# alexkeroro86/SampleNeRFRO

Hardware: AMD Instinct MI355X
Metric: rays/sec (train step) (higher is better)
Workload: dtype f16x3/fp32-acc

## Files before the change

samplenerfro_amd/csrc/mlp.hip:

```cpp
#include "common.h"
#include "nerfmlp_layout.h"
#include "mfma_ops.h"
#include "bkgd_layout.h"
#include "so3_layout.h"

#include <stdlib.h>
#include <type_traits>
#include <vector>
#include <stdio.h>

namespace rnerf {


#define GLOBAL_AS __attribute__((address_space(1)))
#define LDS_AS __attribute__((address_space(3)))

struct MfmaLayer { int dense, ks, nt, kind; };
__host__ __device__ constexpr MfmaLayer mfma_layer(int l) {
  constexpr MfmaLayer t[10] = {{0, 4, 8, 0},  {1, 16, 8, 1}, {2, 16, 8, 1}, {3, 16, 8, 1}, {4, 16, 8, 1},
                               {5, 20, 8, 2}, {6, 16, 8, 1}, {7, 16, 8, 1}, {9, 16, 8, 1}, {10, 18, 4, 3}};
  return t[l];
}
__host__ __device__ constexpr int layer_blocks_before(int l) {
  int o = 0;
// ... 374 lines not shown
template <int PREC, bool MASK, bool ONE = false>
struct SeamWork {
  f32x16 (&acc0)[8];
  f32x16 (&acc1)[8];
  f32x16 (&prev0)[8];
  float4* st1;
  PrevConv<PREC, 0, MASK, true, ONE> cv;
  __device__ __forceinline__ SeamWork(f32x16 (&a0)[8], f32x16 (&a1)[8], f32x16 (&p0)[8], float4* s1) : acc0(a0), acc1(a1), prev0(p0), st1(s1), cv(a0[0]) {}
  template <int C, int T>
  __device__ __forceinline__ void move() {
    if constexpr (C == 0) prev0[T] = acc0[T];
    else if constexpr (!ONE) st1[(T * 4 + C - 1) * 64] = make_float4(acc1[T][4 * (C - 1)], acc1[T][4 * (C - 1) + 1], acc1[T][4 * (C - 1) + 2], acc1[T][4 * (C - 1) + 3]);
  }
  template <int C, int Q>
  __device__ __forceinline__ void conv() {
    if constexpr (ONE && Q >= 4) return;
    if constexpr (C == 0 && Q >= 4) { cv.v1[2 * (Q & 3)] = acc1[0][2 * (Q & 3)]; cv.v1[2 * (Q & 3) + 1] = acc1[0][2 * (Q & 3) + 1]; }
    cv.template chunk<C, Q>();
  }
  template <int C, int PI>
  __device__ __forceinline__ void chunk() {
    if constexpr (PI >= 1) {
      move<C, PI - 1>();
      conv<C, PI - 1>();
      if constexpr (PI == 7 && C == 4) { conv<0, 7>(); conv<1, 7>(); conv<2, 7>(); conv<3, 7>(); conv<4, 7>(); }
    }
  }
  __device__ __forceinline__ void finish() {
    move<0, 7>(); move<1, 7>(); move<2, 7>(); move<3, 7>(); move<4, 7>();
  }
};


template <int PREC, bool FIRST, int PI, typename W, int PASSES = Prec<PREC>::PASSES, typename BOPS = KOps>
__device__ __forceinline__ void tile_mfma(f32x16& a0, f32x16& a1, const uint4 ah, const uint4 al, const BOPS& b, W& work) {
  using PP = Prec<PREC>;
  constexpr bool TWO = !BOPS::ONE;
  const f32x16 zero = {0, 0, 0, 0, 0, 0, 0, 0, 0, 0, 0, 0, 0, 0, 0, 0};
  a0 = mfma16<PP::F16>(ah, b.h0, FIRST ? zero : a0);
  work.template chunk<0, PI>();
  RNERF_PIN();
  if constexpr (TWO) a1 = mfma16<PP::F16>(ah, b.h1, FIRST ? zero : a1);
  work.template chunk<1, PI>();
  RNERF_PIN();
  if constexpr (PP::NP == 2 && PASSES == 3) {
    a0 = mfma16<PP::F16>(ah, b.l0, a0);
    work.template chunk<2, PI>();
    RNERF_PIN();
    if constexpr (TWO) a1 = mfma16<PP::F16>(ah, b.l1, a1);
    work.template chunk<3, PI>();
    RNERF_PIN();
    a0 = mfma16<PP::F16>(al, b.h0, a0);
    work.template chunk<4, PI>();
    RNERF_PIN();
    if constexpr (TWO) a1 = mfma16<PP::F16>(al, b.h1, a1);
  } else if constexpr (PP::NP == 2 && PASSES == 38) {
    a0 = mfma_f8(al.x, al.y, b.l0.x, b.l0.y, a0);
    work.template chunk<2, PI>();
    RNERF_PIN();
    if constexpr (TWO) a1 = mfma_f8(al.x, al.y, b.l1.x, b.l1.y, a1);
    work.template chunk<3, PI>();
    RNERF_PIN();
    a0 = mfma_f8(al.z, al.w, b.l0.z, b.l0.w, a0);
    work.template chunk<4, PI>();
    RNERF_PIN();
    if constexpr (TWO) a1 = mfma_f8(al.z, al.w, b.l1.z, b.l1.w, a1);
  } else if constexpr (PP::NP == 2 && PASSES == 2) {
    a0 = mfma16<PP::F16>(ah, b.l0, a0);
    work.template chunk<2, PI>();
    work.template chunk<3, PI>();
    RNERF_PIN();
    if constexpr (TWO) a1 = mfma16<PP::F16>(ah, b.l1, a1);
    work.template chunk<4, PI>();
  } else if constexpr (PP::NP == 2 && PASSES == 22) {
    a0 = mfma16<PP::F16>(al, b.h0, a0);
    work.template chunk<2, PI>();
    work.template chunk<3, PI>();
    RNERF_PIN();
    if constexpr (TWO) a1 = mfma16<PP::F16>(al, b.h1, a1);
    work.template chunk<4, PI>();
  } else {
    work.template chunk<2, PI>();
    work.template chunk<3, PI>();
    work.template chunk<4, PI>();
  }
  RNERF_PIN();
}

struct NoDma { __device__ __forceinline__ void operator()() const {} };

constexpr int FRAG_DEPTH = 4;

template <int PREC, int NT, int KOFF, bool FIRST, typename W, typename D = NoDma, int PASSES = Prec<PREC>::PASSES, typename BOPS = KOps>
__device__ __forceinline__ void kstep_mfma(f32x16 (&acc0)[8], f32x16 (&acc1)[8], const BOPS& b, const char* slab, int lane, W& work, D dma = D()) {
  using PP = Prec<PREC>;
  const uint4* a = (const uint4*)slab + lane + (size_t)KOFF * NT * PP::NP * 64;
  uint4 fh[FRAG_DEPTH], fl[FRAG_DEPTH];
  auto load_lo = [&](int tile) -> uint4 {
    if constexpr (PP::F8X) {
      const uint2* a2 = (const uint2*)((const uint4*)slab + ((size_t)KOFF * NT + tile) * PP::NP * 64 + 64) + lane;
      const uint2 u = a2[0], v = a2[64];
      return make_uint4(u.x, u.y, v.x, v.y);
    } else return a[(tile * PP::NP + PP::NP - 1) * 64];
  };
#pragma unroll
  for (int t = 0; t < FRAG_DEPTH; ++t) {
    const int tt = t < NT ? t : NT - 1;
    fh[t] = a[(tt * PP::NP) * 64];
    fl[t] = load_lo(tt);
  }
#define RNERF_TILE(T)                                                                                     \
  if constexpr (T < NT) {                                                                                 \
    const uint4 ah = fh[T % FRAG_DEPTH], al = fl[T % FRAG_DEPTH];                                         \
    tile_mfma<PREC, FIRST, (T & 7), W, PASSES, BOPS>(acc0[T], acc1[T], ah, al, b, work);                  \
    if constexpr (T + FRAG_DEPTH < NT) {                                                                  \
      fh[T % FRAG_DEPTH] = a[((T + FRAG_DEPTH) * PP::NP) * 64];                                           \
      fl[T % FRAG_DEPTH] = load_lo(T + FRAG_DEPTH);                                                       \
    }                                                                                                     \
  }
  RNERF_TILE(0) RNERF_TILE(1)
  dma();
  RNERF_TILE(2)
  if constexpr (NT == 8) RNERF_PIN();
  RNERF_TILE(3)
  if constexpr (NT == 8) RNERF_PIN();
  RNERF_TILE(4)
  if constexpr (NT == 8) RNERF_PIN();
  RNERF_TILE(5)
  if constexpr (NT == 8) RNERF_PIN();
  RNERF_TILE(6) RNERF_TILE(7)
#undef RNERF_TILE
}

constexpr int SAVE_PE = 0, SAVE_L1 = 4, SAVE_VIEW = 148, SAVE_RGBIN = 150, SAVE_SLOTS = 158, SAVE_MASK = 158, SAVE_TOTAL = 167;
__host__ __device__ constexpr size_t sv_mask0(long long R) { return (size_t)(R / 32) * SAVE_SLOTS * 64; }
__host__ __device__ constexpr size_t sv_lo0(long long R) { return sv_mask0(R) + (size_t)(R / 32) * 576; }
__host__ __device__ constexpr size_t sv_addr(int q, long long t32, int m, int h) { return (((size_t)t32 * SAVE_SLOTS + q) * 32 + m) * 2 + h; }
__host__ __device__ constexpr size_t sv_mask_addr(int sw, long long t32, int m, int h) { return (((size_t)t32 * 36 + sw) * 32 + m) * 2 + h; }

__device__ __forceinline__ uint32_t nz_nibbles(const uint4& o) {
  return pk_min1(o.x) | (pk_min1(o.y) << 1) | (pk_min1(o.z) << 2) | (pk_min1(o.w) << 3);
}
__device__ __forceinline__ uint32_t nz_byte(uint32_t nib) { return (nib & 0xFu) | (nib >> 12); }

template <int PREC, int MODE, int TRAIN, bool ONE = false>
__global__ void __launch_bounds__(256, 1)
nerfmlp_fwd_kernel(const char* __restrict__ packed, const float4* __restrict__ rows_pd, const float4* __restrict__ rows_dr,
// ... 44 lines not shown
      return n_tiles;
    } else {
      return t;
    }
  };
  const int first_tile = find_next((int)blockIdx.x);
  if (first_tile < n_tiles) { issue_slab<SLAB>(packed, 0u, wave, lane); off = SLAB; }
  slab_wait_dma();
  __syncthreads();

  for (int tile = first_tile; tile < n_tiles;) {
    if (tileq != nullptr && tid == 0)
      __hip_atomic_store(tileq + 1 + blockIdx.x, (int)gridDim.x + atomicAdd(tileq, 1), __ATOMIC_RELAXED, __HIP_MEMORY_SCOPE_AGENT);
    const float* __restrict__ auxt = aux;
    asm volatile("" : "+s"(auxt));
    int next_tile = n_tiles;
    long long row[2]; bool row_ok[2];
    float4 pd[2], dr[2];
#pragma unroll
    for (int mt = 0; mt < 2; ++mt) {
      if (ONE && mt == 1) { row[1] = row[0]; row_ok[1] = false; pd[1] = pd[0]; dr[1] = dr[0]; continue; }
      row[mt] = (long long)tile * TROWS + wave * WROWS + mt * 32 + m;
      row_ok[mt] = row[mt] < total_rows;
      if (!row_ok[mt]) row[mt] = total_rows - 1;
      size_t rec = (size_t)row[mt];
      if (node_of_sample) { const long long sidx = row[mt] / B; rec = (size_t)node_of_sample[sidx] * B + (size_t)(row[mt] - sidx * B); }
      pd[mt] = rows_pd[rec];
      dr[mt] = rows_dr[rec];
    }

    f32x16 acc0[8], acc1[8], prev0[8];

    const long long t32_0 = (long long)tile * (TROWS / 32) + wave * (WROWS / 32);
    auto save_ops = [&](int q, const KOps& o) {
      if constexpr (TRAIN != 0) {
        uint4* dst = save + sv_addr(q, t32_0, m, h);
        stream_store(dst, o.h0);
        if constexpr (!ONE) stream_store(dst + (size_t)SAVE_SLOTS * 64, o.h1);
        if constexpr (TRAIN == 2) {
          uint4* dl = dst + sv_lo0(save_rows);
          stream_store(dl, o.l0);
          if constexpr (!ONE) stream_store(dl + (size_t)SAVE_SLOTS * 64, o.l1);
        }
        if constexpr (TRAIN == 3) {
          uint2* dl = (uint2*)(save + sv_lo0(save_rows)) + sv_addr(q, t32_0, m, h);
          stream_store8(dl, lo8_pack<false>(o.l0, LO8_SCALE_X));
          if constexpr (!ONE) stream_store8(dl + (size_t)SAVE_SLOTS * 64, lo8_pack<false>(o.l1, LO8_SCALE_X));
        }
      }
    };

    uint32_t ovf0 = 0, ovf1 = 0;
    auto watch = [&](const KOps& o, bool is_signed) {
      const uint32_t am = is_signed ? 0x7FFF7FFFu : 0xFFFFFFFFu;
      ovf0 = pk_maxu(pk_maxu(ovf0, o.h0.x & am), pk_maxu(pk_maxu(o.h0.y & am, o.h0.z & am), o.h0.w & am));
      if constexpr (!ONE) ovf1 = pk_maxu(pk_maxu(ovf1, o.h1.x & am), pk_maxu(pk_maxu(o.h1.y & am, o.h1.z & am), o.h1.w & am));
    };

    uint32_t mw0 = 0, mw1 = 0;
    auto save_mask = [&](int set, int s, uint32_t nib0, uint32_t nib1) {
      if constexpr (TRAIN != 0) {
        if ((s & 3) == 0) { mw0 = nz_byte(nib0); mw1 = nz_byte(nib1); }
        else { mw0 |= nz_byte(nib0) << (8 * (s & 3)); mw1 |= nz_byte(nib1) << (8 * (s & 3)); }
        if ((s & 3) == 3) {
          uint32_t* dst = (uint32_t*)(save + sv_mask0(save_rows)) + sv_mask_addr(set * 4 + (s >> 2), t32_0, m, h);
          __builtin_nontemporal_store(mw0, dst);
          if constexpr (!ONE) __builtin_nontemporal_store(mw1, dst + 36 * 64);
        }
      }
    };

    auto enc_ops = [&](const float4 (&v)[2], int s, int nsin) -> KOps {
      const float phase = h ? 1.5707963705062866f : 0.0f;
      float f[2][8];
#pragma unroll
      for (int mt = 0; mt < (ONE ? 1 : 2); ++mt)
#pragma unroll
        for (int j = 0; j < 8; ++j) {
          const int q = 8 * s + j;
          if (q < nsin) {
            const int d = q / 3, c = q % 3;
            const float x = c == 0 ? v[mt].x : (c == 1 ? v[mt].y : v[mt].z);
            f[mt][j] = pe_sin(fadd(fmul(x, (float)(1 << d)), phase));
// ... 23 lines not shown
      }
      KOps o;
      split8<PREC>(x0, o.h0, o.l0);
      if constexpr (ONE) { o.h1 = o.h0; o.l1 = o.l0; } else split8<PREC>(x1, o.h1, o.l1);
      return o;
    };

    auto load_bias8 = [&](int s, const float* __restrict__ bias, float (&b)[8]) {
      const float4 b0 = *(const float4*)(bias + 16 * s + 4 * h), b1 = *(const float4*)(bias + 16 * s + 8 + 4 * h);
      b[0] = b0.x; b[1] = b0.y; b[2] = b0.z; b[3] = b0.w; b[4] = b1.x; b[5] = b1.y; b[6] = b1.z; b[7] = b1.w;
    };
    auto load_state8 = [&](int s, float (&v)[8]) {
      if constexpr (ONE) return;
      const float4 u0 = st1[((s >> 1) * 4 + 2 * (s & 1)) * 64], u1 = st1[((s >> 1) * 4 + 2 * (s & 1) + 1) * 64];
      v[0] = u0.x; v[1] = u0.y; v[2] = u0.z; v[3] = u0.w; v[4] = u1.x; v[5] = u1.y; v[6] = u1.z; v[7] = u1.w;
    };
    NoWork nowork;

#define SLAB_PREFETCH(DO_NEXT)                                                                                       \
  do { if (DO_NEXT) { issue_slab<SLAB>(packed + off, (unsigned)((buf ^ 1) * SLAB), wave, lane); off += SLAB; } } while (0)
#define SLAB_DONE() do { slab_wait_dma(); __syncthreads(); buf ^= 1; } while (0)

    float sig0 = 0.f, sig1 = 0.f;

    KOps cur;
    {
      cur = enc_ops(pd, 0, 30);
      SeamWork<PREC, TRAIN != 0, ONE> seam(acc0, acc1, prev0, st1);
      seam.cv.floor_v = RELU_FLOOR;
      load_bias8(0, auxt + AUX_BIAS, seam.cv.b);
      load_bias8(0, auxt + AUX_ZERO, seam.cv.ws);
#define RNERF_PE_KSTEP(S, FIRST_, SAVE_)                                                                             \
      {                                                                                                              \
        if (SAVE_) save_ops(SAVE_PE + S, cur);                                                                       \
        watch(cur, true);          \
        SLAB_PREFETCH(true);    \
        if constexpr (S < 3) {                                                                                       \
          EncWork<PREC, S + 1, 30, ONE> ew(pd, h);                                                                        \
          kstep_mfma<PREC, 8, 0, FIRST_>(acc0, acc1, cur, smem + buf * SLAB, lane, ew);                              \
          cur = ew.result();                                                                                         \
        } else {                                                                                                     \
          kstep_mfma<PREC, 8, 0, false>(acc0, acc1, cur, smem + buf * SLAB, lane, seam);                             \
        }                                                                                                            \
        SLAB_DONE();                                                                                                 \
      }
      RNERF_PE_KSTEP(0, true, true) RNERF_PE_KSTEP(1, false, true) RNERF_PE_KSTEP(2, false, true) RNERF_PE_KSTEP(3, false, true)
      seam.finish();
      cur = seam.cv.result();
    }

    float bnext[8], wnext[8];
    load_bias8(1, auxt + AUX_BIAS, bnext);
    load_bias8(1, auxt + AUX_ZERO, wnext);

#pragma unroll 1
    for (int l = 1; l <= 8; ++l) {
      const float* __restrict__ bias = auxt + AUX_BIAS + 256 * (l - 1);
      SeamWork<PREC, TRAIN != 0, ONE> seam(acc0, acc1, prev0, st1);
      seam.cv.floor_v = l == 8 ? NO_FLOOR : RELU_FLOOR;
      const float* __restrict__ wseam = auxt + (l == 7 ? AUX_WSIG : AUX_ZERO);
      const float* __restrict__ wsel = auxt + (l == 8 ? AUX_WSIG : AUX_ZERO);
#define RNERF_KSTEP(S)                                                                                              \
      {                                                                                                              \
        save_ops(SAVE_L1 + 16 * (l - 1) + S, cur);                                                                   \
        watch(cur, false);                                                                                           \
        if constexpr (TRAIN != 0 && S == 0) save_mask(l - 1, 0, nz_nibbles(cur.h0), nz_nibbles(cur.h1));                  \
        if constexpr (S == 13) { load_bias8(0, bias + 256, seam.cv.b); load_bias8(0, wseam, seam.cv.ws); }           \
        float bnn[8], wnn[8];                                                                                        \
        if constexpr (S + 2 < 16) { load_bias8(S + 2, bias, bnn); load_bias8(S + 2, wsel, wnn); }    \
        else if constexpr (S == 14) { load_bias8(1, bias + 256, bnn); load_bias8(1, wseam, wnn); }    \
        auto dma = [&]() { SLAB_PREFETCH(true); };                                                                   \
        if constexpr (S + 1 < 16) {                                                                                  \
          PrevConv<PREC, S + 1, TRAIN != 0, true, ONE> cv(prev0[(S + 1) >> 1]);                                           \
          cv.floor_v = RELU_FLOOR;                                                                                        \
          _Pragma("unroll") for (int j = 0; j < 8; ++j) { cv.b[j] = bnext[j]; cv.ws[j] = wnext[j]; }                 \
          load_state8(S + 1, cv.v1);                                                                                 \
          kstep_mfma<PREC, 8, 0, S == 0, PrevConv<PREC, S + 1, TRAIN != 0, true, ONE>, decltype(dma)>(acc0, acc1, cur, smem + buf * SLAB, lane, cv, dma); \
          cur = cv.result();                                                                                         \
          sig0 += cv.sg0; sig1 += cv.sg1;                                                                            \
          save_mask(l - 1, S + 1, cv.nz[0], cv.nz[1]);                                                               \
        } else {                                                                                                     \
           \
           \
          kstep_mfma<PREC, 8, 0, false, SeamWork<PREC, TRAIN != 0, ONE>, decltype(dma)>(acc0, acc1, cur, smem + buf * SLAB, lane, seam, dma); \
        }                                                                                                            \
        if constexpr (S + 2 <= 16) { _Pragma("unroll") for (int j = 0; j < 8; ++j) { bnext[j] = bnn[j]; wnext[j] = wnn[j]; } } \
        SLAB_DONE();                                                                                                 \
      }
      RNERF_KSTEP(0) RNERF_KSTEP(1) RNERF_KSTEP(2) RNERF_KSTEP(3) RNERF_KSTEP(4) RNERF_KSTEP(5) RNERF_KSTEP(6) RNERF_KSTEP(7)
      RNERF_KSTEP(8) RNERF_KSTEP(9) RNERF_KSTEP(10) RNERF_KSTEP(11) RNERF_KSTEP(12) RNERF_KSTEP(13) RNERF_KSTEP(14) RNERF_KSTEP(15)
#undef RNERF_KSTEP
      if (l == 5) {
        asm volatile("" : "+v"(pd[0].x), "+v"(pd[0].y), "+v"(pd[0].z), "+v"(pd[1].x), "+v"(pd[1].y), "+v"(pd[1].z));
        cur = enc_ops(pd, 0, 30);
        RNERF_PE_KSTEP(0, false, false) RNERF_PE_KSTEP(1, false, false) RNERF_PE_KSTEP(2, false, false) RNERF_PE_KSTEP(3, false, false)
      }
      seam.finish();
      cur = seam.cv.result();
      sig0 += seam.cv.sg0; sig1 += seam.cv.sg1;
    }

    {
      const float* __restrict__ bias = auxt + AUX_BIAS + 256 * 8;
      KOps c0 = cur;
      KOps c1 = prev_ops(1, bias, NO_FLOOR);
      float bA[8], bB[8];
      load_bias8(2, bias, bA);
      load_bias8(3, bias, bB);
#define RNERF_VSLAB(SL)                                                                                              \
      {                                                                                                              \
        save_ops(SAVE_L1 + 16 * 8 + 2 * SL, c0);                                                                     \
        save_ops(SAVE_L1 + 16 * 8 + 2 * SL + 1, c1);                                                                 \
        watch(c0, true); watch(c1, true);                                                                            \
        SLAB_PREFETCH(true);                                                                                         \
        if constexpr (SL + 1 < 8) {                                                                                  \
          float bA2[8], bB2[8];                                                                                      \
          if constexpr (SL + 2 < 8) { load_bias8(2 * SL + 4, bias, bA2); load_bias8(2 * SL + 5, bias, bB2); }        \
          PrevConv<PREC, 2 * SL + 2, false, false, ONE> cvA(prev0[SL + 1]);                                                      \
          PrevConv<PREC, 2 * SL + 3, false, false, ONE> cvB(prev0[SL + 1]);                                                      \
          cvA.floor_v = NO_FLOOR; cvB.floor_v = NO_FLOOR;                                                                \
          _Pragma("unroll") for (int j = 0; j < 8; ++j) { cvA.b[j] = bA[j]; cvB.b[j] = bB[j]; }                      \
          load_state8(2 * SL + 2, cvA.v1);                                                                           \
          load_state8(2 * SL + 3, cvB.v1);                                                                           \
          PairOfPairs<decltype(cvA)> wA(cvA);                                                                        \
          PairOfPairs<decltype(cvB)> wB(cvB);                                                                        \
          kstep_mfma<PREC, 4, 0, SL == 0>(acc0, acc1, c0, smem + buf * SLAB, lane, wA);                              \
          kstep_mfma<PREC, 4, 1, false>(acc0, acc1, c1, smem + buf * SLAB, lane, wB);                                \
          c0 = cvA.result(); c1 = cvB.result();                                                                      \
          if constexpr (SL + 2 < 8) { _Pragma("unroll") for (int j = 0; j < 8; ++j) { bA[j] = bA2[j]; bB[j] = bB2[j]; } } \
        } else {                                                                                                     \
          const KOps n0 = enc_ops(dr, 0, 12), n1 = enc_ops(dr, 1, 12);                                               \
          kstep_mfma<PREC, 4, 0, false>(acc0, acc1, c0, smem + buf * SLAB, lane, nowork);                            \
          kstep_mfma<PREC, 4, 1, false>(acc0, acc1, c1, smem + buf * SLAB, lane, nowork);                            \
          c0 = n0; c1 = n1;                                                                                          \
        }                                                                                                            \
        SLAB_DONE();                                                                                                 \
      }
      RNERF_VSLAB(0) RNERF_VSLAB(1) RNERF_VSLAB(2) RNERF_VSLAB(3) RNERF_VSLAB(4) RNERF_VSLAB(5) RNERF_VSLAB(6) RNERF_VSLAB(7)
#undef RNERF_VSLAB
      save_ops(SAVE_VIEW, c0);
      save_ops(SAVE_VIEW + 1, c1);
      watch(c0, true); watch(c1, true);
      next_tile = tileq != nullptr ? __builtin_amdgcn_readfirstlane(__hip_atomic_load(tileq + 1 + blockIdx.x, __ATOMIC_RELAXED, __HIP_MEMORY_SCOPE_AGENT))
                                   : find_next(tile + (int)gridDim.x);
      const bool has_next_tile = next_tile < n_tiles;
      if (has_next_tile) off = 0;
      SLAB_PREFETCH(has_next_tile);
      kstep_mfma<PREC, 4, 0, false>(acc0, acc1, c0, smem + buf * SLAB, lane, nowork);
      kstep_mfma<PREC, 4, 1, false>(acc0, acc1, c1, smem + buf * SLAB, lane, nowork);
      SLAB_DONE();
    }

    {
      const float* __restrict__ hw = auxt + 4 * h;
      auto head_load = [&](int t, float4 (&W)[16]) {
#pragma unroll
        for (int g = 0; g < 4; ++g) {
          const int n = 32 * t + 8 * g;
          W[4 * g] = gload4(hw + AUX_BIAS + 256 * 9 + n);
          W[4 * g + 1] = gload4(hw + AUX_WRGB + n); W[4 * g + 2] = gload4(hw + AUX_WRGB + 128 + n); W[4 * g + 3] = gload4(hw + AUX_WRGB + 256 + n);
        }
      };
      float p0[3] = {0.f, 0.f, 0.f}, p1[3] = {0.f, 0.f, 0.f};
      float4 Wc[16];
      head_load(0, Wc);
#pragma unroll
      for (int t = 0; t < 4; ++t) {
        float4 Wn[16];
        if (t + 1 < 4) head_load(t + 1, Wn);
        RNERF_PIN();
        float rv0[16], rv1[16];
#pragma unroll
        for (int g = 0; g < 4; ++g) {
          const float4 bb = Wc[4 * g], wr = Wc[4 * g + 1], wg = Wc[4 * g + 2], wb = Wc[4 * g + 3];
          const float bv[4] = {bb.x, bb.y, bb.z, bb.w}, wrv[4] = {wr.x, wr.y, wr.z, wr.w}, wgv[4] = {wg.x, wg.y, wg.z, wg.w}, wbv[4] = {wb.x, wb.y, wb.z, wb.w};
#pragma unroll
          for (int i = 0; i < 4; ++i) {
            const float v0 = relu_keep(fmaf(acc0[t][4 * g + i], INV_SCALE, bv[i]), RELU_FLOOR);
            p0[0] = fmaf(v0, wrv[i], p0[0]); p0[1] = fmaf(v0, wgv[i], p0[1]); p0[2] = fmaf(v0, wbv[i], p0[2]);
            rv0[4 * g + i] = v0;
            if constexpr (!ONE) {
              const float v1 = relu_keep(fmaf(acc1[t][4 * g + i], INV_SCALE, bv[i]), RELU_FLOOR);
// ... 174 lines not shown
  int buf = 0;
  size_t off = 0;
  NoWork nowork;

  if ((int)blockIdx.x < n_tiles) { issue_slab<SLAB>(packed_bwd, 0u, wave, lane); off = SLAB; }
  slab_wait_dma();
  __syncthreads();

  float mref = 0.f;
  for (int tile = blockIdx.x; tile < n_tiles; tile += gridDim.x) {
    const bool has_next_tile = tile + (int)gridDim.x < n_tiles;
    const long long srow0 = (long long)tile * TROWS + wave * WROWS + m;
    const long long t32_0 = (long long)tile * (TROWS / 32) + wave * (WROWS / 32);
    float4 g[2];
#pragma unroll
    for (int mt = 0; mt < 2; ++mt) {
      if (ONE && mt == 1) { g[1] = make_float4(0.f, 0.f, 0.f, 0.f); continue; }
      const long long row = srow0 + 32 * mt;
      g[mt] = row < total_rows ? d_raw[row] : make_float4(0.f, 0.f, 0.f, 0.f);
      if constexpr (BW::F16) {
        const float mx = fmaxf(fmaxf(fabsf(g[mt].x), fabsf(g[mt].y)), fmaxf(fabsf(g[mt].z), fabsf(g[mt].w)));
        const uint32_t ex = __builtin_bit_cast(uint32_t, mx) >> 23;
        const bool okx = ex >= 8 && ex <= 250;
        const float m_row = okx ? __builtin_bit_cast(float, (ex - 5) << 23) : 0.0f;
        const float inv = okx ? __builtin_bit_cast(float, (259 - ex) << 23) : 0.0f;
        g[mt].x *= inv; g[mt].y *= inv; g[mt].z *= inv; g[mt].w *= inv;
        float* rs = (float*)(dy + dy_plane_uint4(save_rows, BW::NP));
        if (h == 0) rs[row] = m_row;
        mref = fmaxf(mref, m_row);
      }
    }
    f32x16 acc0[8], acc1[8], prev0[8];

    auto dy_store = [&](int q, const KOps& o) {
      uint4* dst = dy + dy_addr(q, t32_0, m, h);
      stream_store(dst, o.h0);
      if constexpr (!ONE) stream_store(dst + (size_t)DY_SLOTS * 64, o.h1);
      if constexpr (BW::LO8) {
        uint2* dl = (uint2*)(dy + dy_plane_uint4(save_rows, 1)) + dy_addr(q, t32_0, m, h);
        stream_store8(dl, lo8_pack<true>(o.l0, LO8_SCALE_D));
        if constexpr (!ONE) stream_store8(dl + (size_t)DY_SLOTS * 64, lo8_pack<true>(o.l1, LO8_SCALE_D));
      } else if constexpr (BW::NP == 2) {
        uint4* dl = dst + dy_plane_uint4(save_rows, 1);
        stream_store(dl, o.l0);
        if constexpr (!ONE) stream_store(dl + (size_t)DY_SLOTS * 64, o.l1);
      }
    };
    auto mask_at = [&](int set, uint4& a, uint4& b) {
      const uint32_t* src = (const uint32_t*)(saved + sv_mask0(save_rows)) + sv_mask_addr(set * 4, t32_0, m, h);
      constexpr size_t ws = 64, mt1 = 36 * 64;
#define RNERF_NTL(P) __builtin_nontemporal_load(P)
      a = make_uint4(RNERF_NTL(src), RNERF_NTL(src + ws), RNERF_NTL(src + 2 * ws), RNERF_NTL(src + 3 * ws));
      if constexpr (ONE) b = make_uint4(0, 0, 0, 0);
      else b = make_uint4(RNERF_NTL(src + mt1), RNERF_NTL(src + ws + mt1), RNERF_NTL(src + 2 * ws + mt1), RNERF_NTL(src + 3 * ws + mt1));
#undef RNERF_NTL
    };
    auto grad_ops = [&](int s, bool use_mask, const uint4 mk0, const uint4 mk1, const float* __restrict__ wadd) -> KOps {
      float r1[8] = {0.f, 0.f, 0.f, 0.f, 0.f, 0.f, 0.f, 0.f};
      if constexpr (!ONE) {
        const float4 u0 = st1[((s >> 1) * 4 + 2 * (s & 1)) * 64], u1 = st1[((s >> 1) * 4 + 2 * (s & 1) + 1) * 64];
        r1[0] = u0.x; r1[1] = u0.y; r1[2] = u0.z; r1[3] = u0.w; r1[4] = u1.x; r1[5] = u1.y; r1[6] = u1.z; r1[7] = u1.w;
      }
      const uint32_t w0 = (s >> 2) == 0 ? mk0.x : ((s >> 2) == 1 ? mk0.y : ((s >> 2) == 2 ? mk0.z : mk0.w));
      const uint32_t w1 = (s >> 2) == 0 ? mk1.x : ((s >> 2) == 1 ? mk1.y : ((s >> 2) == 2 ? mk1.z : mk1.w));
      float x0[8], x1[8];
#pragma unroll
      for (int j = 0; j < 8; ++j) {
        float a = prev0[s >> 1][8 * (s & 1) + j] * INV_SCALE, b = r1[j] * INV_SCALE;
        if (wadd) { const float w = wadd[16 * s + 8 * (j >> 2) + 4 * h + (j & 3)]; a = fmaf(g[0].w, w, a); b = fmaf(g[1].w, w, b); }
        if (use_mask) {
          const uint32_t bit = 1u << (8 * (s & 3) + (j >> 1) + 4 * (j & 1));
          a = (w0 & bit) ? a : 0.f;
          b = (w1 & bit) ? b : 0.f;
        }
        x0[j] = a; x1[j] = b;
      }
      KOps o;
      if constexpr (ONE) { split8<PREC>(x0, o.h0, o.l0); if constexpr (!(NEED_LO || BW::NP == 2)) o.l0 = make_uint4(0, 0, 0, 0); o.h1 = o.h0; o.l1 = o.l0; }
      else if constexpr (NEED_LO || BW::NP == 2) { split8<PREC>(x0, o.h0, o.l0); split8<PREC>(x1, o.h1, o.l1); }
// ... 19 lines not shown
  do { if (DO_NEXT) { issue_slab<SLAB>(packed_bwd + off, (unsigned)((buf ^ 1) * SLAB), wave, lane); off += SLAB; } } while (0)
#define SLAB_DONE() do { slab_wait_dma(); __syncthreads(); buf ^= 1; } while (0)

    {
      KOps o;
      float hz0[8] = {0, 0, 0, 0, 0, 0, 0, 0}, hz1[8] = {0, 0, 0, 0, 0, 0, 0, 0};
      if (h == 0) { hz0[0] = g[0].w; hz0[1] = g[0].x; hz0[2] = g[0].y; hz0[3] = g[0].z; hz1[0] = g[1].w; hz1[1] = g[1].x; hz1[2] = g[1].y; hz1[3] = g[1].z; }
      split8<PREC>(hz0, o.h0, o.l0);
      if constexpr (ONE) { o.h1 = o.h0; o.l1 = o.l0; } else split8<PREC>(hz1, o.h1, o.l1);
      dy_store(DY_HEADS, o);
#pragma unroll
      for (int t = 0; t < 8; ++t)
#pragma unroll
        for (int r = 0; r < 16; ++r) {
          float a = 0.f, b = 0.f;
          if (t < 4) {
            const int n = 32 * t + (r & 3) + 8 * (r >> 2) + 4 * h;
            const float wr = fwd_aux[AUX_WRGB + n], wg = fwd_aux[AUX_WRGB + 128 + n], wb = fwd_aux[AUX_WRGB + 256 + n];
            a = (g[0].x * wr + g[0].y * wg + g[0].z * wb) * PP::WSCALE;
            b = (g[1].x * wr + g[1].y * wg + g[1].z * wb) * PP::WSCALE;
          }
          acc0[t][r] = a;
          if constexpr (!ONE) acc1[t][r] = b;
        }
      layer_end();
    }

    {
      uint4 ma, mb;
      mask_at(8, ma, mb);
      KOps cur = grad_ops(0, true, ma, mb, nullptr);
#define RNERF_DG_KSTEP(S, NSTEPS, SLOT0, PREFETCH_STMT)                                                                       \
      {                                                                                                                         \
        dy_store((SLOT0) + S, cur);                                                                                             \
        auto dma = [&]() { PREFETCH_STMT; };    \
        if constexpr (S + 1 < NSTEPS) {                                                                                         \
          GradConv<PREC, S + 1, NEED_LO, ONE> cv(prev0[(S + 1) >> 1]);                                                                   \
          if constexpr (!ONE) {                                                                                                 \
            const float4 u0 = st1[(((S + 1) >> 1) * 4 + 2 * ((S + 1) & 1)) * 64], u1 = st1[(((S + 1) >> 1) * 4 + 2 * ((S + 1) & 1) + 1) * 64]; \
            cv.v1[0] = u0.x; cv.v1[1] = u0.y; cv.v1[2] = u0.z; cv.v1[3] = u0.w; cv.v1[4] = u1.x; cv.v1[5] = u1.y; cv.v1[6] = u1.z; cv.v1[7] = u1.w; \
          }                                                                                                                     \
          if (wadd) {            \
            const float4 wa = *(const float4*)(wadd + 16 * (S + 1) + 4 * h), wb = *(const float4*)(wadd + 16 * (S + 1) + 8 + 4 * h); \
            const float wv[8] = {wa.x, wa.y, wa.z, wa.w, wb.x, wb.y, wb.z, wb.w};                                               \
            _Pragma("unroll") for (int j = 0; j < 8; ++j) { cv.t0[j] = g[0].w * wv[j]; cv.t1[j] = g[1].w * wv[j]; }             \
          } else {                                                                                                              \
            _Pragma("unroll") for (int j = 0; j < 8; ++j) { cv.t0[j] = 0.f; cv.t1[j] = 0.f; }                                   \
          }                                                                                                                     \
          cv.w0 = ((S + 1) >> 2) == 0 ? ma.x : (((S + 1) >> 2) == 1 ? ma.y : (((S + 1) >> 2) == 2 ? ma.z : ma.w));             \
          cv.w1 = ((S + 1) >> 2) == 0 ? mb.x : (((S + 1) >> 2) == 1 ? mb.y : (((S + 1) >> 2) == 2 ? mb.z : mb.w));             \
          kstep_mfma<PREC, 8, 0, S == 0, GradConv<PREC, S + 1, NEED_LO, ONE>, decltype(dma), DGP>(acc0, acc1, cur, smem + buf * SLAB, lane, cv, dma); \
          cur = cv.result();                                                                                                    \
        } else {                                                                                                                \
          kstep_mfma<PREC, 8, 0, false, NoWork, decltype(dma), DGP>(acc0, acc1, cur, smem + buf * SLAB, lane, nowork, dma);         \
        }                                                                                                                       \
        SLAB_DONE();                                                                                                            \
      }
      {
        const float* __restrict__ wadd = nullptr;
        RNERF_DG_KSTEP(0, 8, DY_L9, SLAB_PREFETCH(true)) RNERF_DG_KSTEP(1, 8, DY_L9, SLAB_PREFETCH(true))
        RNERF_DG_KSTEP(2, 8, DY_L9, SLAB_PREFETCH(true)) RNERF_DG_KSTEP(3, 8, DY_L9, SLAB_PREFETCH(true))
        RNERF_DG_KSTEP(4, 8, DY_L9, SLAB_PREFETCH(true)) RNERF_DG_KSTEP(5, 8, DY_L9, SLAB_PREFETCH(true))
        RNERF_DG_KSTEP(6, 8, DY_L9, SLAB_PREFETCH(true)) RNERF_DG_KSTEP(7, 8, DY_L9, SLAB_PREFETCH(true))
      }
      layer_end();
    }

    uint4 nma = make_uint4(0, 0, 0, 0), nmb = nma;
#pragma unroll 1
    for (int l = 8; l >= 1; --l) {
      const bool use_mask = l != 8;
      const float* __restrict__ wadd = (l == 7) ? fwd_aux + AUX_WSIG : nullptr;
      uint4 ma = nma, mb = nmb;
      if (!use_mask) { ma = make_uint4(~0u, ~0u, ~0u, ~0u); mb = ma; }
      mask_at(l - 1, nma, nmb);
      KOps cur = grad_ops(0, true, ma, mb, wadd);
      const int slot0 = 16 * l;
#define RNERF_DG_PF(S) do { if ((S) == 15 && l == 1) { if (has_next_tile) off = 0; SLAB_PREFETCH(has_next_tile); } else SLAB_PREFETCH(true); } while (0)
      RNERF_DG_KSTEP(0, 16, slot0, RNERF_DG_PF(0)) RNERF_DG_KSTEP(1, 16, slot0, RNERF_DG_PF(1)) RNERF_DG_KSTEP(2, 16, slot0, RNERF_DG_PF(2))
      RNERF_DG_KSTEP(3, 16, slot0, RNERF_DG_PF(3)) RNERF_DG_KSTEP(4, 16, slot0, RNERF_DG_PF(4)) RNERF_DG_KSTEP(5, 16, slot0, RNERF_DG_PF(5))
      RNERF_DG_KSTEP(6, 16, slot0, RNERF_DG_PF(6)) RNERF_DG_KSTEP(7, 16, slot0, RNERF_DG_PF(7)) RNERF_DG_KSTEP(8, 16, slot0, RNERF_DG_PF(8))
      RNERF_DG_KSTEP(9, 16, slot0, RNERF_DG_PF(9)) RNERF_DG_KSTEP(10, 16, slot0, RNERF_DG_PF(10)) RNERF_DG_KSTEP(11, 16, slot0, RNERF_DG_PF(11))
      RNERF_DG_KSTEP(12, 16, slot0, RNERF_DG_PF(12)) RNERF_DG_KSTEP(13, 16, slot0, RNERF_DG_PF(13)) RNERF_DG_KSTEP(14, 16, slot0, RNERF_DG_PF(14))
      RNERF_DG_KSTEP(15, 16, slot0, RNERF_DG_PF(15))
#undef RNERF_DG_PF
      layer_end();
    }
// ... 1913 lines not shown
```

Baseline: 673,900.

## Stagger activation save stores across MFMA slots, one wave per slot

Instead of issuing all operand/gradient save stores for a k-step as a burst before the MFMA sequence, the stores are split into parts and scheduled at distinct MFMA positions inside the k-step. Each part is issued by only one wave, chosen by MFMA position, so the waves take turns rather than all storing at the same time. A static check keeps a store from sharing a slot with the weight DMA. The aim is to spread global write traffic across the matrix pipeline and reduce store-queue stalls. The cost is more template machinery and a different per-lane address computation, and correctness depends on every store part landing at some slot.

Result: slower. 643,100 (-4.6%).

```diff
diff --git a/samplenerfro_amd/csrc/mlp.hip b/samplenerfro_amd/csrc/mlp.hip
--- a/samplenerfro_amd/csrc/mlp.hip
+++ b/samplenerfro_amd/csrc/mlp.hip
@@ -430,52 +430,87 @@
 };
 
 
-template <int PREC, bool FIRST, int PI, typename W, int PASSES = Prec<PREC>::PASSES, typename BOPS = KOps>
-__device__ __forceinline__ void tile_mfma(f32x16& a0, f32x16& a1, const uint4 ah, const uint4 al, const BOPS& b, W& work) {
+struct NoSave {
+  template <int POS, int M> static constexpr bool stores_at() { return false; }
+  template <int POS, int M> __device__ __forceinline__ void at() const {}
+};
+template <int J> struct StorePart { static constexpr int value = J; };
+template <int NS, typename F>
+struct StaggeredSave {
+  const int wave;
+  const F store;
+  __device__ __forceinline__ StaggeredSave(int wave_, const F& store_) : wave(wave_), store(store_) {}
+  template <int POS, int M> static constexpr bool stores_at() { return POS % (M / NS / 4) == 0 && (POS % (M / NS)) / (M / NS / 4) < 4; }
+  template <int POS, int M> __device__ __forceinline__ void at() const {
+    static_assert(M % NS == 0 && M / NS >= 4, "fewer than four MFMAs per store");
+    if constexpr (stores_at<POS, M>()) {
+      if (wave == (POS % (M / NS)) / (M / NS / 4)) store(StorePart<POS / (M / NS)>());
+    }
+  }
+};
+template <int NS, typename F>
+__device__ __forceinline__ StaggeredSave<NS, F> staggered_save(int wave, const F& store) { return StaggeredSave<NS, F>(wave, store); }
+
+template <int PREC, int PASSES, bool ONE>
+constexpr int tile_mfmas() {
+  constexpr int per = Prec<PREC>::NP != 2 ? 1 : ((PASSES == 3 || PASSES == 38) ? 3 : ((PASSES == 2 || PASSES == 22) ? 2 : 1));
+  return per * (ONE ? 1 : 2);
+}
+
+template <int PREC, bool FIRST, int PI, typename W, int PASSES = Prec<PREC>::PASSES, typename BOPS = KOps, typename SV = NoSave, int T = 0, int NT = 8>
+__device__ __forceinline__ void tile_mfma(f32x16& a0, f32x16& a1, const uint4 ah, const uint4 al, const BOPS& b, W& work, const SV& sv = SV()) {
   using PP = Prec<PREC>;
   constexpr bool TWO = !BOPS::ONE;
+  constexpr int MPT = tile_mfmas<PREC, PASSES, BOPS::ONE>(), M = NT * MPT, P0 = T * MPT, ST = TWO ? 2 : 1;
   const f32x16 zero = {0, 0, 0, 0, 0, 0, 0, 0, 0, 0, 0, 0, 0, 0, 0, 0};
   a0 = mfma16<PP::F16>(ah, b.h0, FIRST ? zero : a0);
+  sv.template at<P0, M>();
   work.template chunk<0, PI>();
   RNERF_PIN();
-  if constexpr (TWO) a1 = mfma16<PP::F16>(ah, b.h1, FIRST ? zero : a1);
+  if constexpr (TWO) { a1 = mfma16<PP::F16>(ah, b.h1, FIRST ? zero : a1); sv.template at<P0 + 1, M>(); }
   work.template chunk<1, PI>();
   RNERF_PIN();
   if constexpr (PP::NP == 2 && PASSES == 3) {
     a0 = mfma16<PP::F16>(ah, b.l0, a0);
+    sv.template at<P0 + ST, M>();
     work.template chunk<2, PI>();
     RNERF_PIN();
-    if constexpr (TWO) a1 = mfma16<PP::F16>(ah, b.l1, a1);
+    if constexpr (TWO) { a1 = mfma16<PP::F16>(ah, b.l1, a1); sv.template at<P0 + 3, M>(); }
     work.template chunk<3, PI>();
     RNERF_PIN();
     a0 = mfma16<PP::F16>(al, b.h0, a0);
+    sv.template at<P0 + 2 * ST, M>();
     work.template chunk<4, PI>();
     RNERF_PIN();
-    if constexpr (TWO) a1 = mfma16<PP::F16>(al, b.h1, a1);
+    if constexpr (TWO) { a1 = mfma16<PP::F16>(al, b.h1, a1); sv.template at<P0 + 5, M>(); }
   } else if constexpr (PP::NP == 2 && PASSES == 38) {
     a0 = mfma_f8(al.x, al.y, b.l0.x, b.l0.y, a0);
+    sv.template at<P0 + ST, M>();
     work.template chunk<2, PI>();
     RNERF_PIN();
-    if constexpr (TWO) a1 = mfma_f8(al.x, al.y, b.l1.x, b.l1.y, a1);
+    if constexpr (TWO) { a1 = mfma_f8(al.x, al.y, b.l1.x, b.l1.y, a1); sv.template at<P0 + 3, M>(); }
     work.template chunk<3, PI>();
     RNERF_PIN();
     a0 = mfma_f8(al.z, al.w, b.l0.z, b.l0.w, a0);
+    sv.template at<P0 + 2 * ST, M>();
     work.template chunk<4, PI>();
     RNERF_PIN();
-    if constexpr (TWO) a1 = mfma_f8(al.z, al.w, b.l1.z, b.l1.w, a1);
+    if constexpr (TWO) { a1 = mfma_f8(al.z, al.w, b.l1.z, b.l1.w, a1); sv.template at<P0 + 5, M>(); }
   } else if constexpr (PP::NP == 2 && PASSES == 2) {
     a0 = mfma16<PP::F16>(ah, b.l0, a0);
+    sv.template at<P0 + ST, M>();
     work.template chunk<2, PI>();
     work.template chunk<3, PI>();
     RNERF_PIN();
-    if constexpr (TWO) a1 = mfma16<PP::F16>(ah, b.l1, a1);
+    if constexpr (TWO) { a1 = mfma16<PP::F16>(ah, b.l1, a1); sv.template at<P0 + 3, M>(); }
     work.template chunk<4, PI>();
   } else if constexpr (PP::NP == 2 && PASSES == 22) {
     a0 = mfma16<PP::F16>(al, b.h0, a0);
+    sv.template at<P0 + ST, M>();
     work.template chunk<2, PI>();
     work.template chunk<3, PI>();
     RNERF_PIN();
-    if constexpr (TWO) a1 = mfma16<PP::F16>(al, b.h1, a1);
+    if constexpr (TWO) { a1 = mfma16<PP::F16>(al, b.h1, a1); sv.template at<P0 + 3, M>(); }
     work.template chunk<4, PI>();
   } else {
     work.template chunk<2, PI>();
@@ -486,12 +521,13 @@
 }
 
 struct NoDma { __device__ __forceinline__ void operator()() const {} };
-
 constexpr int FRAG_DEPTH = 4;
 
-template <int PREC, int NT, int KOFF, bool FIRST, typename W, typename D = NoDma, int PASSES = Prec<PREC>::PASSES, typename BOPS = KOps>
-__device__ __forceinline__ void kstep_mfma(f32x16 (&acc0)[8], f32x16 (&acc1)[8], const BOPS& b, const char* slab, int lane, W& work, D dma = D()) {
+template <int PREC, int NT, int KOFF, bool FIRST, typename W, typename D = NoDma, int PASSES = Prec<PREC>::PASSES, typename BOPS = KOps, typename SV = NoSave>
+__device__ __forceinline__ void kstep_mfma(f32x16 (&acc0)[8], f32x16 (&acc1)[8], const BOPS& b, const char* slab, int lane, W& work, D dma = D(), const SV& sv = SV()) {
   using PP = Prec<PREC>;
+  static_assert(std::is_same<D, NoDma>::value || !SV::template stores_at<2 * tile_mfmas<PREC, PASSES, BOPS::ONE>() - 1, NT * tile_mfmas<PREC, PASSES, BOPS::ONE>()>(),
+                "an operand save shares its place with the weight DMA");
   const uint4* a = (const uint4*)slab + lane + (size_t)KOFF * NT * PP::NP * 64;
   uint4 fh[FRAG_DEPTH], fl[FRAG_DEPTH];
   auto load_lo = [&](int tile) -> uint4 {
@@ -510,7 +546,7 @@
 #define RNERF_TILE(T)                                                                                     \
   if constexpr (T < NT) {                                                                                 \
     const uint4 ah = fh[T % FRAG_DEPTH], al = fl[T % FRAG_DEPTH];                                         \
-    tile_mfma<PREC, FIRST, (T & 7), W, PASSES, BOPS>(acc0[T], acc1[T], ah, al, b, work);                  \
+    tile_mfma<PREC, FIRST, (T & 7), W, PASSES, BOPS, SV, T, NT>(acc0[T], acc1[T], ah, al, b, work, sv);   \
     if constexpr (T + FRAG_DEPTH < NT) {                                                                  \
       fh[T % FRAG_DEPTH] = a[((T + FRAG_DEPTH) * PP::NP) * 64];                                           \
       fl[T % FRAG_DEPTH] = load_lo(T + FRAG_DEPTH);                                                       \
@@ -621,23 +657,25 @@
     f32x16 acc0[8], acc1[8], prev0[8];
 
     const long long t32_0 = (long long)tile * (TROWS / 32) + wave * (WROWS / 32);
+    const unsigned lane16_ = (unsigned)(m * 2 + h) * 16u;
+    constexpr int SAVE_MT = ONE ? 1 : 2, SAVE_NS = SAVE_MT * (TRAIN >= 2 ? 2 : 1);
+    auto save_part = [&](int q, const KOps& o, auto J) {
+      constexpr int plane = decltype(J)::value / SAVE_MT, mt = decltype(J)::value % SAVE_MT;
+      if constexpr (TRAIN != 0) {
+        const size_t blk = sv_addr(q, t32_0 + mt, 0, 0);
+        unsigned lane16 = lane16_;
+        asm volatile("" : "+v"(lane16));
+        if constexpr (plane == 0) stream_store((uint4*)((char*)(save + blk) + lane16), mt ? o.h1 : o.h0);
+        else if constexpr (TRAIN == 2) stream_store((uint4*)((char*)(save + sv_lo0(save_rows) + blk) + lane16), mt ? o.l1 : o.l0);
+        else stream_store8((uint2*)((char*)((uint2*)(save + sv_lo0(save_rows)) + blk) + lane16 / 2), lo8_pack<false>(mt ? o.l1 : o.l0, LO8_SCALE_X));
+      }
+    };
     auto save_ops = [&](int q, const KOps& o) {
-      if constexpr (TRAIN != 0) {
-        uint4* dst = save + sv_addr(q, t32_0, m, h);
-        stream_store(dst, o.h0);
-        if constexpr (!ONE) stream_store(dst + (size_t)SAVE_SLOTS * 64, o.h1);
-        if constexpr (TRAIN == 2) {
-          uint4* dl = dst + sv_lo0(save_rows);
-          stream_store(dl, o.l0);
-          if constexpr (!ONE) stream_store(dl + (size_t)SAVE_SLOTS * 64, o.l1);
-        }
-        if constexpr (TRAIN == 3) {
-          uint2* dl = (uint2*)(save + sv_lo0(save_rows)) + sv_addr(q, t32_0, m, h);
-          stream_store8(dl, lo8_pack<false>(o.l0, LO8_SCALE_X));
-          if constexpr (!ONE) stream_store8(dl + (size_t)SAVE_SLOTS * 64, lo8_pack<false>(o.l1, LO8_SCALE_X));
-        }
-      }
+      save_part(q, o, StorePart<0>());
+      if constexpr (SAVE_NS >= 2) save_part(q, o, StorePart<1>());
+      if constexpr (SAVE_NS == 4) { save_part(q, o, StorePart<2>()); save_part(q, o, StorePart<3>()); }
     };
+    const int save_wave = TRAIN != 0 ? wave : -1;
 
     uint32_t ovf0 = 0, ovf1 = 0;
     auto watch = [&](const KOps& o, bool is_signed) {
@@ -727,15 +765,15 @@
       load_bias8(0, auxt + AUX_ZERO, seam.cv.ws);
 #define RNERF_PE_KSTEP(S, FIRST_, SAVE_)                                                                             \
       {                                                                                                              \
-        if (SAVE_) save_ops(SAVE_PE + S, cur);                                                                       \
+        auto sv = staggered_save<SAVE_NS>((SAVE_) ? save_wave : -1, [&](auto J) { save_part(SAVE_PE + S, cur, J); });   \
         watch(cur, true);          \
         SLAB_PREFETCH(true);    \
         if constexpr (S < 3) {                                                                                       \
           EncWork<PREC, S + 1, 30, ONE> ew(pd, h);                                                                        \
-          kstep_mfma<PREC, 8, 0, FIRST_>(acc0, acc1, cur, smem + buf * SLAB, lane, ew);                              \
+          kstep_mfma<PREC, 8, 0, FIRST_>(acc0, acc1, cur, smem + buf * SLAB, lane, ew, NoDma(), sv);                 \
           cur = ew.result();                                                                                         \
         } else {                                                                                                     \
-          kstep_mfma<PREC, 8, 0, false>(acc0, acc1, cur, smem + buf * SLAB, lane, seam);                             \
+          kstep_mfma<PREC, 8, 0, false>(acc0, acc1, cur, smem + buf * SLAB, lane, seam, NoDma(), sv);                \
         }                                                                                                            \
         SLAB_DONE();                                                                                                 \
       }
@@ -757,7 +795,7 @@
       const float* __restrict__ wsel = auxt + (l == 8 ? AUX_WSIG : AUX_ZERO);
 #define RNERF_KSTEP(S)                                                                                              \
       {                                                                                                              \
-        save_ops(SAVE_L1 + 16 * (l - 1) + S, cur);                                                                   \
+        auto sv = staggered_save<SAVE_NS>(save_wave, [&](auto J) { save_part(SAVE_L1 + 16 * (l - 1) + S, cur, J); });  \
         watch(cur, false);                                                                                           \
         if constexpr (TRAIN != 0 && S == 0) save_mask(l - 1, 0, nz_nibbles(cur.h0), nz_nibbles(cur.h1));                  \
         if constexpr (S == 13) { load_bias8(0, bias + 256, seam.cv.b); load_bias8(0, wseam, seam.cv.ws); }           \
@@ -770,14 +808,14 @@
           cv.floor_v = RELU_FLOOR;                                                                                        \
           _Pragma("unroll") for (int j = 0; j < 8; ++j) { cv.b[j] = bnext[j]; cv.ws[j] = wnext[j]; }                 \
           load_state8(S + 1, cv.v1);                                                                                 \
-          kstep_mfma<PREC, 8, 0, S == 0, PrevConv<PREC, S + 1, TRAIN != 0, true, ONE>, decltype(dma)>(acc0, acc1, cur, smem + buf * SLAB, lane, cv, dma); \
+          kstep_mfma<PREC, 8, 0, S == 0, PrevConv<PREC, S + 1, TRAIN != 0, true, ONE>, decltype(dma), PP::PASSES, KOps>(acc0, acc1, cur, smem + buf * SLAB, lane, cv, dma, sv); \
           cur = cv.result();                                                                                         \
           sig0 += cv.sg0; sig1 += cv.sg1;                                                                            \
           save_mask(l - 1, S + 1, cv.nz[0], cv.nz[1]);                                                               \
         } else {                                                                                                     \
            \
            \
-          kstep_mfma<PREC, 8, 0, false, SeamWork<PREC, TRAIN != 0, ONE>, decltype(dma)>(acc0, acc1, cur, smem + buf * SLAB, lane, seam, dma); \
+          kstep_mfma<PREC, 8, 0, false, SeamWork<PREC, TRAIN != 0, ONE>, decltype(dma), PP::PASSES, KOps>(acc0, acc1, cur, smem + buf * SLAB, lane, seam, dma, sv); \
         }                                                                                                            \
         if constexpr (S + 2 <= 16) { _Pragma("unroll") for (int j = 0; j < 8; ++j) { bnext[j] = bnn[j]; wnext[j] = wnn[j]; } } \
         SLAB_DONE();                                                                                                 \
@@ -804,8 +842,8 @@
       load_bias8(3, bias, bB);
 #define RNERF_VSLAB(SL)                                                                                              \
       {                                                                                                              \
-        save_ops(SAVE_L1 + 16 * 8 + 2 * SL, c0);                                                                     \
-        save_ops(SAVE_L1 + 16 * 8 + 2 * SL + 1, c1);                                                                 \
+        auto sv0 = staggered_save<SAVE_NS>(save_wave, [&](auto J) { save_part(SAVE_L1 + 16 * 8 + 2 * SL, c0, J); });     \
+        auto sv1 = staggered_save<SAVE_NS>(save_wave, [&](auto J) { save_part(SAVE_L1 + 16 * 8 + 2 * SL + 1, c1, J); }); \
         watch(c0, true); watch(c1, true);                                                                            \
         SLAB_PREFETCH(true);                                                                                         \
         if constexpr (SL + 1 < 8) {                                                                                  \
@@ -819,30 +857,30 @@
           load_state8(2 * SL + 3, cvB.v1);                                                                           \
           PairOfPairs<decltype(cvA)> wA(cvA);                                                                        \
           PairOfPairs<decltype(cvB)> wB(cvB);                                                                        \
-          kstep_mfma<PREC, 4, 0, SL == 0>(acc0, acc1, c0, smem + buf * SLAB, lane, wA);                              \
-          kstep_mfma<PREC, 4, 1, false>(acc0, acc1, c1, smem + buf * SLAB, lane, wB);                                \
+          kstep_mfma<PREC, 4, 0, SL == 0>(acc0, acc1, c0, smem + buf * SLAB, lane, wA, NoDma(), sv0);                \
+          kstep_mfma<PREC, 4, 1, false>(acc0, acc1, c1, smem + buf * SLAB, lane, wB, NoDma(), sv1);                  \
           c0 = cvA.result(); c1 = cvB.result();                                                                      \
           if constexpr (SL + 2 < 8) { _Pragma("unroll") for (int j = 0; j < 8; ++j) { bA[j] = bA2[j]; bB[j] = bB2[j]; } } \
         } else {                                                                                                     \
           const KOps n0 = enc_ops(dr, 0, 12), n1 = enc_ops(dr, 1, 12);                                               \
-          kstep_mfma<PREC, 4, 0, false>(acc0, acc1, c0, smem + buf * SLAB, lane, nowork);                            \
-          kstep_mfma<PREC, 4, 1, false>(acc0, acc1, c1, smem + buf * SLAB, lane, nowork);                            \
+          kstep_mfma<PREC, 4, 0, false>(acc0, acc1, c0, smem + buf * SLAB, lane, nowork, NoDma(), sv0);              \
+          kstep_mfma<PREC, 4, 1, false>(acc0, acc1, c1, smem + buf * SLAB, lane, nowork, NoDma(), sv1);              \
           c0 = n0; c1 = n1;                                                                                          \
         }                                                                                                            \
         SLAB_DONE();                                                                                                 \
       }
       RNERF_VSLAB(0) RNERF_VSLAB(1) RNERF_VSLAB(2) RNERF_VSLAB(3) RNERF_VSLAB(4) RNERF_VSLAB(5) RNERF_VSLAB(6) RNERF_VSLAB(7)
 #undef RNERF_VSLAB
-      save_ops(SAVE_VIEW, c0);
-      save_ops(SAVE_VIEW + 1, c1);
+      auto sv0 = staggered_save<SAVE_NS>(save_wave, [&](auto J) { save_part(SAVE_VIEW, c0, J); });
+      auto sv1 = staggered_save<SAVE_NS>(save_wave, [&](auto J) { save_part(SAVE_VIEW + 1, c1, J); });
       watch(c0, true); watch(c1, true);
       next_tile = tileq != nullptr ? __builtin_amdgcn_readfirstlane(__hip_atomic_load(tileq + 1 + blockIdx.x, __ATOMIC_RELAXED, __HIP_MEMORY_SCOPE_AGENT))
                                    : find_next(tile + (int)gridDim.x);
       const bool has_next_tile = next_tile < n_tiles;
       if (has_next_tile) off = 0;
       SLAB_PREFETCH(has_next_tile);
-      kstep_mfma<PREC, 4, 0, false>(acc0, acc1, c0, smem + buf * SLAB, lane, nowork);
-      kstep_mfma<PREC, 4, 1, false>(acc0, acc1, c1, smem + buf * SLAB, lane, nowork);
+      kstep_mfma<PREC, 4, 0, false>(acc0, acc1, c0, smem + buf * SLAB, lane, nowork, NoDma(), sv0);
+      kstep_mfma<PREC, 4, 1, false>(acc0, acc1, c1, smem + buf * SLAB, lane, nowork, NoDma(), sv1);
       SLAB_DONE();
     }
 
@@ -1083,19 +1121,21 @@
     }
     f32x16 acc0[8], acc1[8], prev0[8];
 
+    const unsigned lane16_ = (unsigned)(m * 2 + h) * 16u;
+    constexpr int DY_MT = ONE ? 1 : 2, DY_NS = DY_MT * BW::NP;
+    auto dy_part = [&](int q, const KOps& o, auto J) {
+      constexpr int plane = decltype(J)::value / DY_MT, mt = decltype(J)::value % DY_MT;
+      const size_t blk = dy_addr(q, t32_0 + mt, 0, 0);
+      unsigned lane16 = lane16_;
+      asm volatile("" : "+v"(lane16));
+      if constexpr (plane == 0) stream_store((uint4*)((char*)(dy + blk) + lane16), mt ? o.h1 : o.h0);
+      else if constexpr (BW::LO8) stream_store8((uint2*)((char*)((uint2*)(dy + dy_plane_uint4(save_rows, 1)) + blk) + lane16 / 2), lo8_pack<true>(mt ? o.l1 : o.l0, LO8_SCALE_D));
+      else stream_store((uint4*)((char*)(dy + dy_plane_uint4(save_rows, 1) + blk) + lane16), mt ? o.l1 : o.l0);
+    };
     auto dy_store = [&](int q, const KOps& o) {
-      uint4* dst = dy + dy_addr(q, t32_0, m, h);
-      stream_store(dst, o.h0);
-      if constexpr (!ONE) stream_store(dst + (size_t)DY_SLOTS * 64, o.h1);
-      if constexpr (BW::LO8) {
-        uint2* dl = (uint2*)(dy + dy_plane_uint4(save_rows, 1)) + dy_addr(q, t32_0, m, h);
-        stream_store8(dl, lo8_pack<true>(o.l0, LO8_SCALE_D));
-        if constexpr (!ONE) stream_store8(dl + (size_t)DY_SLOTS * 64, lo8_pack<true>(o.l1, LO8_SCALE_D));
-      } else if constexpr (BW::NP == 2) {
-        uint4* dl = dst + dy_plane_uint4(save_rows, 1);
-        stream_store(dl, o.l0);
-        if constexpr (!ONE) stream_store(dl + (size_t)DY_SLOTS * 64, o.l1);
-      }
+      dy_part(q, o, StorePart<0>());
+      if constexpr (DY_NS >= 2) dy_part(q, o, StorePart<1>());
+      if constexpr (DY_NS == 4) { dy_part(q, o, StorePart<2>()); dy_part(q, o, StorePart<3>()); }
     };
     auto mask_at = [&](int set, uint4& a, uint4& b) {
       const uint32_t* src = (const uint32_t*)(saved + sv_mask0(save_rows)) + sv_mask_addr(set * 4, t32_0, m, h);
@@ -1181,7 +1221,7 @@
       KOps cur = grad_ops(0, true, ma, mb, nullptr);
 #define RNERF_DG_KSTEP(S, NSTEPS, SLOT0, PREFETCH_STMT)                                                                       \
       {                                                                                                                         \
-        dy_store((SLOT0) + S, cur);                                                                                             \
+        auto sv = staggered_save<DY_NS>(wave, [&](auto J) { dy_part((SLOT0) + S, cur, J); });                                   \
         auto dma = [&]() { PREFETCH_STMT; };    \
         if constexpr (S + 1 < NSTEPS) {                                                                                         \
           GradConv<PREC, S + 1, NEED_LO, ONE> cv(prev0[(S + 1) >> 1]);                                                                   \
@@ -1198,10 +1238,10 @@
           }                                                                                                                     \
           cv.w0 = ((S + 1) >> 2) == 0 ? ma.x : (((S + 1) >> 2) == 1 ? ma.y : (((S + 1) >> 2) == 2 ? ma.z : ma.w));             \
           cv.w1 = ((S + 1) >> 2) == 0 ? mb.x : (((S + 1) >> 2) == 1 ? mb.y : (((S + 1) >> 2) == 2 ? mb.z : mb.w));             \
-          kstep_mfma<PREC, 8, 0, S == 0, GradConv<PREC, S + 1, NEED_LO, ONE>, decltype(dma), DGP>(acc0, acc1, cur, smem + buf * SLAB, lane, cv, dma); \
+          kstep_mfma<PREC, 8, 0, S == 0, GradConv<PREC, S + 1, NEED_LO, ONE>, decltype(dma), DGP, KOps>(acc0, acc1, cur, smem + buf * SLAB, lane, cv, dma, sv); \
           cur = cv.result();                                                                                                    \
         } else {                                                                                                                \
-          kstep_mfma<PREC, 8, 0, false, NoWork, decltype(dma), DGP>(acc0, acc1, cur, smem + buf * SLAB, lane, nowork, dma);         \
+          kstep_mfma<PREC, 8, 0, false, NoWork, decltype(dma), DGP, KOps>(acc0, acc1, cur, smem + buf * SLAB, lane, nowork, dma, sv); \
         }                                                                                                                       \
         SLAB_DONE();                                                                                                            \
       }
```
